# vpc-ccg/freddie

Hardware: AMD Instinct MI355X
Metric: reads segmented/sec (whole node) (higher is better)
Workload: dtype u32

## Files before the change

freddie_amd/_lib.py:

```python
import ctypes
import os

import numpy as np

from . import build as _build

_lib = None


class SegError(RuntimeError):

    def __init__(self, msg, code=None):
        super().__init__(msg)
        self.code = code


ERR_ARG, ERR_HIP, ERR_INPUT, ERR_UNSUPPORTED = 1, 2, 3, 4


class _Params(ctypes.Structure):
    _fields_ = [
        ("sigma", ctypes.c_double), ("threshold_rate", ctypes.c_double), ("variance_factor", ctypes.c_double),
        ("max_problem_size", ctypes.c_int32), ("min_read_support_outside", ctypes.c_int32),
        ("ignore_ends", ctypes.c_int32),
# ... 9 lines not shown
        ("part_iv_off", ctypes.c_void_p), ("iv_start", ctypes.c_void_p), ("iv_end", ctypes.c_void_p),
        ("part_rep_off", ctypes.c_void_p), ("rep_weight", ctypes.c_void_p), ("rep_exon_off", ctypes.c_void_p),
        ("ex_ts", ctypes.c_void_p), ("ex_te", ctypes.c_void_p),
    ]


class _Sizes(ctypes.Structure):
    _fields_ = [("n_final", ctypes.c_int64), ("label_bytes", ctypes.c_int64), ("n_cand", ctypes.c_int64),
                ("n_problems", ctypes.c_int64), ("n_positions", ctypes.c_int64), ("max_problem_size", ctypes.c_int64),
                ("max_problem_reads", ctypes.c_int64)]


class _Reads(ctypes.Structure):
    _fields_ = [("n_read", ctypes.c_int64)] + [(k, ctypes.c_void_p) for k in (
        "read_part", "read_rep", "strand", "seq_len", "seq_off", "read_q_off", "qs", "qe", "cig_off", "cig_op", "cig_len", "seq_classes")]


READS_DTYPES = dict(read_part=np.int32, read_rep=np.int32, strand=np.uint8, seq_len=np.int32, seq_off=np.int64, read_q_off=np.int64,
                    qs=np.int32, qe=np.int32, cig_off=np.int64, cig_op=np.uint8, cig_len=np.int32, seq_classes=np.uint32)


class _Annot(ctypes.Structure):
    _fields_ = [("n_read", ctypes.c_int64)] + [(k, ctypes.c_void_p) for k in (
        "gap_off", "gaps", "clip_off", "clips", "poly_off", "polys", "tail", "tok_off", "tok")]


EXPORTS = ["fseg_annotate", "fseg_annotation", "fseg_abi_version", "fseg_source_hash", "fseg_results", "fseg_results_packed", "fseg_create", "fseg_destroy", "fseg_last_error", "fseg_set_params", "fseg_upload",
           "fseg_run", "fseg_sync", "fseg_get_sizes", "fseg_download", "fseg_tap", "fseg_set_profiling",
           "fseg_n_stages", "fseg_stage_name", "fseg_stage_ms", "fseg_scoring_algorithmic_bytes"]

PATHS = ("small_batch", "tiny_on", "wave_on", "fuse_on", "key32", "thr_part", "label_packed", "n_solve0", "n_solve1", "n_solve2",
         "n_wide0", "n_wide1", "n_wide2", "n_tiny", "n_work", "dpw", "wide16", "known", "solve8", "tiny_kernel", "score", "arena_dp",
         "plan", "n_arena_prob", "n_score0", "n_score1", "n_score2", "hist16", "iv_threads", "smooth_r", "yraw16", "thr_chain",
         "lane_sort")

TAPS = dict(pos_off=(1, np.int64), y_raw=(2, np.int32), y=(3, np.float64), threshold=(4, np.float64),
            cand_off=(5, np.int64), cand_y=(6, np.int32), fixed=(7, np.uint8), chosen=(8, np.uint8),
            final_off=(9, np.int64), final_y=(10, np.int32), problems=(11, np.int32),
            lane_start=(12, np.int32), lane_pmax=(13, np.int32), lane_exons=(14, np.int64),
            lane_stream=(15, np.int32), exon_stream=(16, np.int32), sync=(17, np.int32), paths=(18, np.int32),
            hist_ranges=(19, np.int64))


def lib_path():
    return os.environ.get("FSEG_LIB") or _build.SEG_SO


def load():
    global _lib
    if _lib is not None:
        return _lib
    path = lib_path()
    if not os.path.exists(path):
        raise SegError("%s not found: build it first (freddie_amd.build.build_seg()); there is no CPU fallback" % path)
    L = ctypes.CDLL(path)
    vp = ctypes.c_void_p
    L.fseg_abi_version.restype = ctypes.c_int
    L.fseg_create.restype = ctypes.c_int
    L.fseg_create.argtypes = [ctypes.c_int, ctypes.POINTER(vp)]
    L.fseg_destroy.restype = None
    L.fseg_destroy.argtypes = [vp]
    L.fseg_last_error.restype = ctypes.c_char_p
    L.fseg_last_error.argtypes = [vp]
    L.fseg_set_params.restype = ctypes.c_int
    L.fseg_set_params.argtypes = [vp, ctypes.POINTER(_Params)]
    L.fseg_upload.restype = ctypes.c_int
    L.fseg_upload.argtypes = [vp, ctypes.POINTER(_Batch)]
# ... 184 lines not shown
```

freddie_amd/csrc/freddie_seg.hip:

```cpp
#include "seg_kernels.h"

using namespace fseg;

namespace {

template <typename T> struct DevBuf {
    T *p = nullptr;
    size_t cap = 0;
    static size_t bytes(size_t n) { return n * sizeof(T); }
};
template <> struct DevBuf<void> {
    void *p = nullptr;
    size_t cap = 0;
    static size_t bytes(size_t n) { return n; }
    template <typename U> U *as() const { return static_cast<U *>(p); }
};
template <typename T> size_t bytes_of(const DevBuf<T> &, size_t n) { return DevBuf<T>::bytes(n); }
struct NoCopy { NoCopy() = default; NoCopy(const NoCopy &) = delete; NoCopy &operator=(const NoCopy &) = delete; };
template <typename T> struct OwnDev : DevBuf<T>, NoCopy {
    ~OwnDev() { if (this->p) (void)hipFree(this->p); }
    hipError_t alloc(size_t bytes) { this->cap = bytes; return hipMalloc(&this->p, bytes); }
};
struct Slab : OwnDev<void> {};
template <typename T> struct Pinned : NoCopy {
// ... 25 lines not shown
                                        "interval_scoring", "dp", "refine", "final_positions", "labels", "graph_pre",
                                        "graph_post"};

enum : unsigned {
    SEG_PRE1 = 1u,
    SEG_PRE2 = 2u,
    SEG_SCORE = 4u,
    SEG_POST1 = 8u,
    SEG_POST2 = 16u,
    SEG_STATUS = 32u,
    SEG_ALL = 63u,
};

}

hipError_t fseg_sort_pairs(void *tmp, size_t *tmp_bytes, const unsigned long long *keys_in, unsigned long long *keys_out,
                           const int *vals_in, int *vals_out, size_t n, unsigned end_bit, hipStream_t stream);

struct fseg_ctx {
    int device = 0;
    hipStream_t stream = nullptr;
    std::string err;
    bool have_params = false, have_batch = false, ran = false, pending = false;
    bool fetched = false;
    fseg_params P{};
    std::vector<double> w_main, w_refine, h_table;
    int n_part = 0;
    i64 K = 0, R = 0, I = 0, NPOS = 0, LANES = 0;
    i64 max_part_pos = 0;
    int thr_part = -1;
    int hist16 = -1;
    bool hist_packed = false;
    int thr_chain = -1;
    int yraw16 = -1;
    bool yraw_narrow = false;
    i64 max_part_lanes = 0;
    int n_tiles = 0;
    bool expanded = false;
    std::vector<i64> part_iv_off, part_rep_off;
    Slab slab_in, slab_pos, slab_arena;
    Pinned<char> h_stage;
    Pinned<char> h_res;
    size_t res_off[4] = {0, 0, 0, 0};
    std::vector<i64> res_pfo;
    OwnDev<void> d_labels;
    OwnDev<unsigned> d_packed;
    int fetched_packed = -1;
    bool label_packed_ok = true;
    bool label_has2 = false;
    bool run_label_packed = false;
    bool labels_unpacked = false;
    OwnDev<void> d_sort_tmp;
    DevBuf<i64> d_part_iv_off, d_part_rep_off, d_part_lane_off, d_pos_off, d_rep_exon_off, d_hc_p0, d_rb_sum, d_rb_base;
    DevBuf<int> d_iv_start, d_iv_end, d_iv_part, d_rep_weight, d_ex_ts, d_ex_te, d_iv_tile0, d_blk_iv0, d_rb_part, d_rb_r0, d_rb_max, d_rb_cmax,
        d_hc_part, d_hc_n, d_hc_glo, d_hc_ghi;
    DevBuf<TileDesc> d_tile_desc;
    DevBuf<longlong2> d_lane_ex;
    DevBuf<int> d_lane_start, d_lane_pmax, d_val_a, d_val_b, d_rep_last;
    DevBuf<i64> d_hc_llo, d_hc_lhi, d_rb_esum, d_rb_ebase;
    DevBuf<u64> d_key_a, d_key_b;
    DevBuf<int2> d_lane_lx, d_lex;
    i64 max_rep_exons = 0;
    OwnDev<double> d_w_main, d_w_refine, d_h_table;
    OwnDev<int2> d_thr_tab;
    DevBuf<unsigned> d_bits;
    DevBuf<void> d_y_raw;
// ... 59 lines not shown
    bool prob_self_scan = false;
    i64 scan_single_max = 512;
    bool force_scan_stall = false;
    hipGraph_t graph[2] = {nullptr, nullptr};
    hipGraphExec_t graph_exec[2] = {nullptr, nullptr};
    bool profile_plain = false;
    int n_graphs = 0;
    bool last_sized = false;
    hipEvent_t ev_b[ST_COUNT] = {}, ev_e[ST_COUNT] = {};
    hipEvent_t ev_g[4] = {};
    float stage_ms[ST_REPORTED] = {};
    static constexpr int kSide = 3, kForkEvents = 32;
    hipStream_t side[kSide] = {};
    hipEvent_t fj[kForkEvents] = {};
    bool use_fork = true;
    bool force_key64 = false;
    bool wide_by_seen = false;
    char score_plan[32] = "gM|W|hB|gST";
    bool use_wave = true;
    bool use_fuse = true;
    int fuse_lanes = kFuseLanesDefault;
    bool wide_solve = true;
    bool fuse_on = true;
    bool counts_known = false;
    i64 n_solve[3] = {0, 0, 0}, n_cls_work[4] = {0, 0, 0, 0}, n_dp_cls[3] = {0, 0, 0}, n_arena_prob = 0, n_tiny = 0;
    i64 n_wide[3] = {0, 0, 0};
    i64 max_ln = 0;
    i64 tiny_from = 256;
    bool trace = false;
    bool force_global_sort = false;
    enum { PATH_SMALL_BATCH, PATH_TINY_ON, PATH_WAVE_ON, PATH_FUSE_ON, PATH_KEY32, PATH_THR_PART, PATH_LABEL_PACKED, PATH_N_SOLVE,
           PATH_N_WIDE = PATH_N_SOLVE + 3, PATH_N_TINY = PATH_N_WIDE + 3, PATH_N_WORK, PATH_DPW, PATH_WIDE16, PATH_KNOWN, PATH_SOLVE8,
           PATH_TINY_KERNEL, PATH_SCORE, PATH_ARENA_DP, PATH_PLAN, PATH_N_ARENA_PROB, PATH_N_SCORE, PATH_HIST16 = PATH_N_SCORE + 3, PATH_IV_THREADS,
           PATH_SMOOTH_R, PATH_YRAW16, PATH_THR_CHAIN, PATH_LANE_SORT, PATH_WORDS };
    int paths[PATH_WORDS] = {};
    OwnDev<void> d_an_in, d_an_work, d_an_out;
    Pinned<char> h_an_in, h_an;
    bool have_annot = false;
    fseg_annot annot{};
    ~fseg_ctx();
};

namespace {

int fail(fseg_ctx *c, int code, const char *fmt, ...) {
    char buf[512];
    va_list ap;
    va_start(ap, fmt);
    vsnprintf(buf, sizeof buf, fmt, ap);
    va_end(ap);
    if (c) c->err = buf;
    if (code == FSEG_ERR_HIP) (void)hipGetLastError();
    return code;
}
thread_local std::string g_create_error;

#define HIP_TRY(c, expr)                                                                         \
    do {                                                                                         \
        hipError_t e__ = (expr);                                                                 \
        if (e__ != hipSuccess) return fail((c), FSEG_ERR_HIP, "%s: %s", #expr, hipGetErrorString(e__)); \
    } while (0)
#define TRY(expr) do { int rc__ = (expr); if (rc__) return rc__; } while (0)

static bool g_ablate_dp = false;
static std::atomic<int> g_in_flight[64];
static std::atomic<int> g_live[64];
static std::atomic<const fseg_ctx *> g_owner[64];
// ... 326 lines not shown
    hipLaunchKernelGGL(k_prob_emit, dim3(pg), dim3(256), 0, s, st, c->d_cand_pn.p, c->d_cand_ll.p,
                       c->d_cand_ln.p, c->d_seg_iv.p, c->d_cand_off.p, prob_bs,
                       pr, c->prob_cap, c->d_work_pc.p, c->d_cls_items.p,
                       c->work_cap, c->d_dp_items.p, c->d_prob_desc.p, c->d_iv_start.p,
                       c->d_iv_part.p, c->d_part_lane_off.p, split, c->d_solve_items.p, c->d_solve_desc.p,
                       c->d_wide_items.p, c->d_wide_all.p, c->d_cand_wide.p,
                       dev_sync ? sw : (SyncWords *)nullptr, sync_gen);
    launch_fork_waiters();
    if (c->prob_cap > 0 && any_arena) {
        if (stage_events && do_score) { end(ST_SCORE_PREP); begin(ST_SCORE); score_begun = true; }
        const int cov_blocks = work_grid < 2048 ? work_grid : 2048;
        const int pt_blocks = c->small_batch ? grid_for(c->prob_cap, 1, 512) : 0;
        if (!pt_blocks)
            hipLaunchKernelGGL(k_pair_thresholds, dim3(grid_for(c->prob_cap, 1, 2048)), dim3(256), 0, s, st, pr,
                               c->d_prob_desc.p, c->prob_cap, c->d_cand_off.p, c->d_cand_y.p,
                               c->d_h_table.p, c->P.h_len,
                               c->P.threshold_rate, c->d_pair_thr.p, c->pair_cap, c->d_amb.p,
                               c->d_out.p, c->tri_cap);
        hipLaunchKernelGGL(k_cov, dim3(cov_blocks + pt_blocks), dim3(kLaneChunk), 0, s, st,
                           c->d_prob_desc.p, c->prob_cap, c->d_work_pc.p, c->work_cap, c->d_cand_off.p,
                           c->d_cand_y.p, c->d_iv_start.p, c->d_lane_lx.p,
                           c->d_lex.p,
                           c->d_cov.p, c->cov_cap, c->d_work_active.p,
                           cov_blocks, pr, c->d_h_table.p, c->P.h_len, c->P.threshold_rate, c->d_pair_thr.p,
                           c->pair_cap, c->d_amb.p, c->d_out.p, c->tri_cap);
    }
    if (!score_begun) end(ST_SCORE_PREP);
    }
    if (do_score && !score_begun) begin(ST_SCORE);
    int *const census = c->paths;
    if (do_score) {
        for (int w = 0; w < fseg_ctx::PATH_WORDS; ++w)
            if (w != fseg_ctx::PATH_THR_PART && w != fseg_ctx::PATH_LABEL_PACKED && w != fseg_ctx::PATH_ARENA_DP && w != fseg_ctx::PATH_HIST16 &&
                w != fseg_ctx::PATH_IV_THREADS && w != fseg_ctx::PATH_SMOOTH_R && w != fseg_ctx::PATH_YRAW16 && w != fseg_ctx::PATH_THR_CHAIN && w != fseg_ctx::PATH_LANE_SORT) census[w] = 0;
        census[fseg_ctx::PATH_SMALL_BATCH] = c->small_batch; census[fseg_ctx::PATH_TINY_ON] = c->tiny_on; census[fseg_ctx::PATH_WAVE_ON] = wave;
        census[fseg_ctx::PATH_FUSE_ON] = c->use_fuse && c->fuse_on; census[fseg_ctx::PATH_KNOWN] = known; census[fseg_ctx::PATH_PLAN] = plan != nullptr;
    }
    if (do_score && c->prob_cap > 0) {
        const bool sfork = any_arena;
        hipStream_t qt = (tiny_max > 0 && sfork) ? fork(2) : s;
#ifdef FSEG_SCORE_TIMING
#define FSEG_TARG , c->d_tacc.p
#else
#define FSEG_TARG
#endif
#ifndef FSEG_WG_SMALL
#define FSEG_WG_SMALL 4096
#endif
#ifndef FSEG_WG_MID
#define FSEG_WG_MID 2048
#endif
#ifndef FSEG_WG_TINY
#define FSEG_WG_TINY 4096
#endif
#define FSEG_LAUNCH_SCORE(Q, NMV, CLS, MAXWG)                                                                           \
        do { note_score(CLS);                                                                                                  \
        hipLaunchKernelGGL(k_score<NMV>, dim3(work_grid < (MAXWG) ? work_grid : (MAXWG)), dim3(ScoreCfg<NMV>::kThreads),  \
                           score_lds_for((NMV) == kNMax ? c->nm_big : (NMV), (NMV) + 1), Q, st, CLS,                                 \
                           ((NMV) == kNMax ? c->nm_big : (NMV)), pr, c->prob_cap, c->d_cls_items.p,              \
                           c->d_prob_desc.p, c->work_cap, c->d_cand_off.p,                         \
                           c->d_cand_y.p, c->d_work_active.p, c->d_cov.p,        \
                           c->cov_cap, c->d_pair_thr.p, c->pair_cap, c->d_out.p, c->tri_cap,      \
                           c->d_amb.p FSEG_TARG); } while (0)
        auto wide_n = [&](int cls, size_t cnt_bytes) -> i64 { return (known && cls >= 0 && cls < 3 && cnt_bytes == 2) ? c->n_wide[cls] : -1; };
#define FSEG_SOLVE_N(CNT, CLS, N_ITEMS) (wide_n(CLS, sizeof(CNT)) >= 0 ? wide_n(CLS, sizeof(CNT)) : (i64)(N_ITEMS))
#define FSEG_SOLVE_WIDE(CNT, CLS) (wide_n(CLS, sizeof(CNT)) >= 0 ? c->d_wide_items.p : (const int *)nullptr)
#define FSEG_SOLVE_ARGS(NMV, CNT, CLS)                                                                                      \
// ... 263 lines not shown
                       c->d_seg_prev.p, c->d_cand_y.p, c->d_pos_off.p, c->d_y_raw.as<COUNT>(), \
                       c->d_w_refine.p, c->P.radius_refine, c->P.sigma, c->d_g.p, c->d_pk.p, \
                       c->d_pf.p, c->d_kp.p, flag_final_bits)
    if (c->yraw_narrow) { FSEG_LAUNCH_REFINE(uint16_t); }
    else { FSEG_LAUNCH_REFINE(int); }
#undef FSEG_LAUNCH_REFINE
    end(ST_REFINE); begin(ST_FINAL);
    pos_counts(s, flag_final_bits);
    hipLaunchKernelGGL(k_scan_emit<kEmitPositions>, dim3(pos_grid), dim3(256), 0, s, flag_final_bits,
                       NPOS, bsum, gsum, scan_state + 2 * scan_nb, &st->n_final, c->d_final_off.p + K, &st->err, (const double *)nullptr, (double *)nullptr, K, c->d_pos_off.p,
                       c->d_iv_start.p, c->d_blk_iv0.p, c->d_final_y.p, c->d_final_pos.p,
                       c->d_final_off.p, 0, c->d_final_iv.p);
    hipLaunchKernelGGL(k_label_cols, dim3(grid_for(NPOS / 8 + 1, 256, 2048)), dim3(256), 0, s, K, c->d_final_off.p,
                       c->d_final_y.p, c->d_final_iv.p, c->d_iv_part.p, c->d_h_table.p, c->P.h_len,
                       c->P.threshold_rate, c->d_thr_tab.p, c->d_col_thr.p, c->d_col_zero.p,
                       c->d_part_has2.p, n_part, c->d_part_iv_off.p, c->d_part_rep_off.p,
                       c->d_label_off.p, st, c->label_cap);
    end(ST_FINAL);
    }
    if (do_post2) {
    begin(ST_LABEL);
    if (c->label_cap > 0) {
        c->run_label_packed = lab_packed; c->labels_unpacked = false;
        c->paths[fseg_ctx::PATH_LABEL_PACKED] = lab_packed;
        if (lab_packed) {
            const i64 n16 = sized ? (label_fill_bytes + 15) / 16 : labels_n16;
            if (n16 > 0)
                hipLaunchKernelGGL(k_clear, dim3(grid_for(n16 / 4 + 1, 256, 4096)), dim3(256), 0, s, (Status *)nullptr, c->d_packed.p, n16);
        } else if (!ride_fill) {
            const i64 n16 = sized ? (label_fill_bytes + 15) / 16 : labels_n16;
            if (n16 > 0)
                hipLaunchKernelGGL(k_label_zero, dim3(grid_for(n16 / 8 + 1, 256, 4096)), dim3(256), 0, s, c->d_labels.as<uint4>(), n16);
        }
        hipLaunchKernelGGL(k_label_reads, dim3(grid_for((i64)c->n_rep_blocks * kLabelSplit, 1, 65536)), dim3(256), 0, s, c->n_rep_blocks,
                           c->d_rb_part.p, c->d_rb_r0.p, c->d_label_off.p, c->label_cap, n_part,
                           c->d_part_iv_off.p, c->d_part_rep_off.p, c->d_final_off.p,
                           c->d_final_pos.p, c->d_col_thr.p, c->d_rep_exon_off.p,
                           c->d_ex_ts.p, c->d_ex_te.p, c->d_col_zero.p,
                           c->d_part_has2.p, c->d_labels.as<unsigned char>(), lab_packed ? c->d_packed.p : (unsigned *)nullptr);
    }
    end(ST_LABEL);
    }
    if (segs & SEG_STATUS) HIP_TRY(c, hipMemcpyAsync(c->h_status.p, st, sizeof(Status), hipMemcpyDeviceToHost, s));
    HIP_TRY(c, fj_err);
    HIP_TRY(c, hipGetLastError());
    return FSEG_OK;
}

hipError_t wait_stream(fseg_ctx *c) {
    const auto t0 = std::chrono::steady_clock::now();
    for (;;) {
        hipError_t e = hipStreamQuery(c->stream);
        if (e != hipErrorNotReady) { (void)hipGetLastError(); return e; }
        if (std::chrono::steady_clock::now() - t0 > std::chrono::milliseconds(2)) break;
    }
    (void)hipGetLastError();
    return hipStreamSynchronize(c->stream);
}

int check_prep(fseg_ctx *c) {
    if (c->prep_checked) return FSEG_OK;
    c->prep_checked = true;
    const PrepStatus &ps = *c->h_prep;
    if (!ps.err) return FSEG_OK;
    int q = 0;
    for (int i = 1; i < 4; ++i) if (((ps.err >> i) & 1u) && (!((ps.err >> q) & 1u) || ps.bad_rep[i] < ps.bad_rep[q])) q = i;
    if (!((ps.err >> q) & 1u)) for (q = 0; q < 4 && !((ps.err >> q) & 1u); ++q) {}
    const long long r = (long long)ps.bad_rep[q];
    c->have_batch = false;
    switch (1u << q) {
        case kPrepExonEnds: return fail(c, FSEG_ERR_INPUT, "rep %lld: exon with start >= end (py/freddie_segment.py:160)", r);
        case kPrepExonOrder: return fail(c, FSEG_ERR_INPUT, "rep %lld: exons out of order (py/freddie_segment.py:158)", r);
// ... 282 lines not shown
        {k_solve<kNMax, unsigned short, int, false>, solve_lds_for(kNMax, kNMax + 1, 2)},
        {k_solve<kNMax, unsigned short, i64, false>, solve_lds_for(kNMax, kNMax + 1, 2)},
        {k_solve<kNMax, unsigned char, int, true>, solve_lds_for(kNMax, kNMax + 1, 1)},
        {k_solve<kNMax, unsigned short, int, true>, solve_lds_for(kNMax, kNMax + 1, 2)},
        {k_dpw<kNMax, unsigned char, int, 64>, dpw_lds_for(kNMax, 4, 1)},
        {k_dpw<kNMax, unsigned short, int, 64>, dpw_lds_for(kNMax, 4, 2)},
        {k_dpw<kNMax, unsigned char, i64, 64>, dpw_lds_for(kNMax, 8, 1)},
        {k_dpw<kNMax, unsigned short, i64, 64>, dpw_lds_for(kNMax, 8, 2)},
        {k_dpw<kNMax, unsigned char, int, 512>, dpw_lds_for(kNMax, 4, 1)},
        {k_dpw<kNMax, unsigned short, int, 512>, dpw_lds_for(kNMax, 4, 2)},
        {k_dpw<kNMax, unsigned char, i64, 512>, dpw_lds_for(kNMax, 8, 1)},
        {k_dpw<kNMax, unsigned short, i64, 512>, dpw_lds_for(kNMax, 8, 2)},
        {k_dp_huge, kHugeDpLds},
    };
    for (const auto &a : lds_attrs) CREATE_TRY(hipFuncSetAttribute(a.fn, hipFuncAttributeMaxDynamicSharedMemorySize, (int)a.bytes));
#undef CREATE_TRY
    return hipSuccess;
}

bool env_flag(const char *name) { const char *v = getenv(name); return v && v[0] == '1'; }
bool env_off(const char *name) { const char *v = getenv(name); return v && v[0] == '0'; }
void env_tri(const char *name, int &out) { const char *v = getenv(name); if (v && (v[0] == '0' || v[0] == '1')) out = v[0] - '0'; }
bool env_int(const char *name, i64 &out) { const char *v = getenv(name); if (!v || !v[0]) return false; out = atoll(v); return true; }
const char *env_str(const char *name) { return getenv(name); }

void read_switches(fseg_ctx *c) {
    i64 v = 0;
    if (env_off("FSEG_DEV_SYNC")) c->dev_sync = false;
    if (env_flag("FSEG_LABEL_BYTES")) c->label_packed_ok = false;
    env_tri("FSEG_THR_PART", c->thr_part);
    env_tri("FSEG_THR_CHAIN", c->thr_chain);
    env_tri("FSEG_HIST16", c->hist16);
    env_tri("FSEG_YRAW16", c->yraw16);
    if (env_int("FSEG_SYNC_TICKS", v) && v > 0) c->sync_ticks = (unsigned)v;
    if (env_flag("FSEG_NO_GRAPH")) c->use_graph = false;
    if (env_flag("FSEG_NO_FORK")) c->use_fork = false;
    if (env_flag("FSEG_NO_FUSE")) c->use_fuse = false;
    if (env_flag("FSEG_NO_WAVE")) c->use_wave = false;
    if (env_flag("FSEG_FORCE_KEY64")) c->force_key64 = true;
    if (env_flag("FSEG_WIDE_BY_SEEN")) c->wide_by_seen = true;
    if (const char *s = env_str("FSEG_SPLIT_DP")) c->split_dp = atoi(s) & 15;
    if (const char *s = env_str("FSEG_SCORE_PLAN")) snprintf(c->score_plan, sizeof c->score_plan, "%s", s);
    {
        int seen[4] = {0, 0, 0, 0};
        static const char kinds[] = "BMST";
        for (const char *q = c->score_plan; *q; ++q) { const char *at = strchr(kinds, *q); if (at) ++seen[at - kinds]; }
        int bars = 0;
        for (const char *q = c->score_plan; *q; ++q) bars += *q == '|';
        if (seen[0] != 1 || seen[1] != 1 || seen[2] != 1 || seen[3] != 1 || bars > fseg_ctx::kSide) c->score_plan[0] = 0;
    }
    if (env_int("FSEG_FUSE_LANES", v) && v > 0 && v <= kFuseLanesWide) c->fuse_lanes = (int)v;
    if (env_flag("FSEG_NO_SIZED")) c->use_sized = false;
    if (env_flag("FSEG_TRACE")) c->trace = true;
    if (env_flag("FSEG_GLOBAL_SORT")) c->force_global_sort = true;
    if (env_flag("FSEG_FORCE_SCAN_STALL")) c->force_scan_stall = true;
    if (env_int("FSEG_TINY_FROM", v)) c->tiny_from = v;
    if (env_int("FSEG_SCAN_SINGLE_MAX", v)) c->scan_single_max = v;
}

}

fseg_ctx::~fseg_ctx() {
    (void)hipSetDevice(device);
    if (stream) (void)hipStreamSynchronize(stream);
    for (hipStream_t q : side) if (q) (void)hipStreamSynchronize(q);
    drop_graph(this);
// ... 934 lines not shown
```

freddie_amd/csrc/seg_common.h:

```cpp
#pragma once
#include <hip/hip_runtime.h>
#include <type_traits>
#include <hsa/hsa.h>
#include <hsa/hsa_ext_amd.h>
#include <chrono>
#include <algorithm>
#include <atomic>
#include <mutex>
#include <cmath>
#include <cstdarg>
#include <cstdio>
#include <cstdlib>
#include <cstring>
#include <string>
#include <vector>

#include "freddie_seg.h"

namespace fseg {


typedef long long i64;

typedef unsigned long long u64;
// ... 1320 lines not shown

constexpr size_t kHugeScoreLds = (size_t)(kNHuge * (kNHuge - 1) / 2) * 8 + (size_t)kHugeSub * (kNHuge + 1) * 4;


constexpr size_t kHugeDpLds = (size_t)(kNHuge * (kNHuge - 1) / 2) * (8 + 4 + 1) + 16;


constexpr int kGiantWgs = 64;

inline size_t giant_score_lds(int nm) { return (size_t)(2 * nm + kHugeSub * (nm + 1)) * 4; }

inline size_t giant_dp_lds(int nm) { return (size_t)nm * 4; }

inline size_t giant_scratch_bytes(int nm) {
    const size_t pairs = (size_t)nm * (nm - 1) / 2;
    return ((pairs * (8 + 4 + 2) + 255) & ~(size_t)255);
}


constexpr int kSegChunks = 4;


constexpr int kRefCap = 1024;

constexpr int kLabelCols = 1024;

#ifndef FSEG_LABEL_STAGE
#define FSEG_LABEL_STAGE 1024
#endif
constexpr int kLabelStage = FSEG_LABEL_STAGE;

constexpr int kLabelSplit = 4;


enum : unsigned { kPrepExonEnds = 1u, kPrepExonOrder = 2u, kPrepExonInterval = 4u, kPrepNoExons = 8u };

struct PrepStatus {
    unsigned err;
    unsigned pad;
    i64 bad_rep[4];
};


constexpr int kLaneSortMax = 2048;

constexpr int kLexChunk = 4096;

__device__ __forceinline__ void lex_copy_tile(int eb, int ne, i64 src0, int tot_e, i64 tile_e0, const int *__restrict__ ex_ts,
                                              const int *__restrict__ ex_te, int2 *__restrict__ lex, unsigned char *owner_s ,
                                              int *eb_s , i64 *src_s ) {
    eb_s[threadIdx.x] = eb; src_s[threadIdx.x] = src0;
    for (int c0 = 0; c0 < tot_e; c0 += kLexChunk) {
        __syncthreads();
        const int lo = max(eb, c0), hi = min(eb + ne, c0 + kLexChunk);
        for (int o = lo; o < hi; ++o) owner_s[o - c0] = (unsigned char)threadIdx.x;
        __syncthreads();
        const int end = min(tot_e, c0 + kLexChunk);
        for (int o = c0 + (int)threadIdx.x; o < end; o += 256) {
            const int u = owner_s[o - c0];
            const i64 src = src_s[u] + (o - eb_s[u]);
            lex[tile_e0 + o] = make_int2(ex_ts[src], ex_te[src]);
        }
    }
    __syncthreads();
}

// ... 12 lines not shown
```

freddie_amd/csrc/seg_kernels.h:

```cpp
#pragma once
#include "seg_common.h"

namespace fseg {

__global__ void __launch_bounds__(256) k_thr_table(const double *h_table, int h_len, double tau, int2 *tab);

template <int BITS, typename Out>
__global__ void __launch_bounds__(512) k_hist(int n_chunks, const int *chunk_part, const i64 *chunk_p0, const int *chunk_n,
                                              const int *chunk_glo, const int *chunk_ghi, const i64 *chunk_lane_lo,
                                              const i64 *chunk_lane_hi, const i64 *part_iv_off,
                                              const int *iv_start, const int *iv_end, const i64 *pos_off,
                                              const i64 *part_lane_off, const int2 *__restrict__ lane_lx, const int *lane_start,
                                              const int *lane_pmax, const int2 *__restrict__ lex,
                                              int ignore_ends, Out *y_raw, Status *st, u64 *zero_ptr, i64 zero_n);

template <int R, typename Count>
#ifndef FSEG_SMOOTH_OCC
#define FSEG_SMOOTH_OCC 6
#endif
__global__ void __launch_bounds__(kSmoothThreads, FSEG_SMOOTH_OCC) k_smooth(int n_tiles, const TileDesc *__restrict__ tiles,
                                                const Count *__restrict__ y_raw, const double *__restrict__ w_g, int radius_rt,
                                                double *y_out, unsigned *flag_pos, unsigned *flag_cand, int *blk_pre, int *tile_tot,
                                                int *tile_defer);

// ... 142 lines not shown

__global__ void __launch_bounds__(512) k_dp_giant(Status *st, const int *dp_items, ProblemArrays pr, const ProbDesc *desc,
                                                  i64 prob_cap, const int *cand_y, const unsigned *out_g, i64 tri_cap,
                                                  const unsigned *amb_g, const int2 *pair_thr, i64 pair_cap, int support,
                                                  unsigned char *chosen, int nm, unsigned char *scratch, i64 scratch_stride);

template <typename Count>
__global__ void k_segments(i64 K, const i64 *pos_off, const i64 *cand_off, const int *cand_y, const Count *__restrict__ y_raw,
                           const int *__restrict__ blk_pre, const int *tile_tot, const int *iv_tile0, const unsigned char *chosen, unsigned *final_flag, int *rseg_c, int *rseg_prev,
                           Status *st);

template <typename Count>
__global__ void __launch_bounds__(64) k_refine(const Status *st, const int *cand_iv, const int *rseg_c,
                                               const int *rseg_prev, const int *cand_y, const i64 *pos_off,
                                               const Count *y_raw, const double *w_g, int radius, double sigma,
                                               double *g_scr, int *pk_scr, unsigned char *flag_scr,
                                               unsigned char *keep_scr, unsigned *final_flag);

__global__ void __launch_bounds__(256) k_label_cols(i64 K, const i64 *final_off, const int *final_y, const int *final_iv, const int *iv_part,
                                                    const double *h_table, int h_len, double tau, const int2 *thr_tab, int2 *col_thr,
                                                    unsigned char *col_zero, int *part_has2, int n_part,
                                                    const i64 *part_iv_off, const i64 *part_rep_off, i64 *label_off,
                                                    Status *st, i64 label_cap);

__global__ void __launch_bounds__(256) k_label_zero(uint4 *labels16, i64 n16);

__global__ void __launch_bounds__(256) k_label_reads(int n_blocks, const int *rb_part, const int *rb_r0,
                                                     const i64 *label_off, i64 label_cap, int n_part,
                                                     const i64 *part_iv_off, const i64 *part_rep_off,
                                                     const i64 *final_off, const int *final_pos, const int2 *col_thr,
                                                     const i64 *rep_exon_off, const int *ex_ts, const int *ex_te,
                                                     const unsigned char *col_zero, const int *part_has2,
                                                     unsigned char *labels, unsigned *packed);
__global__ void __launch_bounds__(256) k_unpack_labels(const unsigned *__restrict__ packed, uint4 *__restrict__ labels16, i64 n16);

__global__ void __launch_bounds__(256) k_pack_labels(const uint4 *__restrict__ labels16, unsigned *__restrict__ packed, i64 n16);

__global__ void __launch_bounds__(256) k_prep_reps(int n_blocks, const int *rb_part, const int *rb_r0, const i64 *part_rep_off,
                                                   const i64 *part_iv_off, const int *iv_start, const int *iv_end,
                                                   const i64 *rep_exon_off, const int *ex_ts, const int *ex_te, u64 *key,
                                                   int *val, int *rep_last, PrepStatus *ps);

__global__ void __launch_bounds__(256) k_lanes(int n_part, const i64 *part_rep_off, const i64 *part_lane_off, const u64 *key_sorted,
                                               const int *val_sorted, const int *rep_weight, const int *rep_last,
                                               const i64 *rep_exon_off, longlong2 *lane_ex, int *lane_start, int *lane_pmax,
                                               int sort_here, const u64 *key_unsorted, const int *ex_ts, const int *ex_te,
                                               int2 *lane_lx, int2 *lex);

__global__ void __launch_bounds__(256) k_lane_blocks(int n_blocks, const int *rb_part, const int *rb_r0, const i64 *part_rep_off,
                                                     const int *val_sorted, const int *rep_weight, const int *rep_last,
                                                     i64 *rb_sum, int *rb_max, const i64 *rep_exon_off, i64 *rb_esum);

__global__ void __launch_bounds__(256) k_lane_block_scan(int n_part, int n_blocks, const int *rb_part, const i64 *part_lane_off,
                                                         const i64 *rb_sum, const int *rb_max, i64 *rb_base, int *rb_cmax,
                                                         const i64 *part_rep_off, const i64 *rep_exon_off, const i64 *rb_esum, i64 *rb_ebase);

__global__ void __launch_bounds__(256) k_lane_emit(int n_blocks, const int *rb_part, const int *rb_r0, const i64 *part_rep_off,
                                                   const u64 *key_sorted, const int *val_sorted, const int *rep_weight, const int *rep_last,
                                                   const i64 *rep_exon_off, const i64 *rb_base, const int *rb_cmax,
                                                   longlong2 *lane_ex, int *lane_start, int *lane_pmax, const i64 *rb_ebase,
                                                   const int *ex_ts, const int *ex_te, int2 *lane_lx, int2 *lex);

__global__ void __launch_bounds__(256) k_hist_ranges(int n_chunks, const int *hc_part, const int *hc_glo, const int *hc_ghi,
                                                     const i64 *part_lane_off, const int *lane_start, const int *lane_pmax,
                                                     i64 *hc_llo, i64 *hc_lhi);

// ... 44 lines not shown
```

freddie_amd/csrc/seg_tail.hip:

```cpp
#include "seg_kernels.h"

namespace fseg {

__device__ __forceinline__ int end_blocks(const int *yr, int a0, int a, int b0, int b) {
    int4u va[kSumBlock / 4], vb[kSumBlock / 4];
#pragma unroll
    for (int e = 0; e < kSumBlock / 4; ++e) { va[e] = *reinterpret_cast<const int4u *>(yr + a0 + 4 * e); vb[e] = *reinterpret_cast<const int4u *>(yr + b0 + 4 * e); }
    int tot = 0;
#pragma unroll
    for (int e = 0; e < kSumBlock / 4; ++e) {
        const int pa = a0 + 4 * e, pb = b0 + 4 * e;
        tot += (pb <= b ? vb[e].x : 0) + (pb + 1 <= b ? vb[e].y : 0) + (pb + 2 <= b ? vb[e].z : 0) + (pb + 3 <= b ? vb[e].w : 0);
        tot -= (pa < a ? va[e].x : 0) + (pa + 1 < a ? va[e].y : 0) + (pa + 2 < a ? va[e].z : 0) + (pa + 3 < a ? va[e].w : 0);
    }
    return tot;
}
__device__ __forceinline__ int end_blocks(const uint16_t *yr, int a0, int a, int b0, int b) {
    uint4u va[kSumBlock / 8], vb[kSumBlock / 8];
#pragma unroll
    for (int e = 0; e < kSumBlock / 8; ++e) { va[e] = *reinterpret_cast<const uint4u *>(yr + a0 + 8 * e); vb[e] = *reinterpret_cast<const uint4u *>(yr + b0 + 8 * e); }
    const int na = a - a0, nb = b - b0 + 1;
    auto first = [](unsigned w, int n) { return n >= 2 ? (w & 0xffffu) + (w >> 16) : (n == 1 ? w & 0xffffu : 0u); };
    unsigned tot_a = 0, tot_b = 0;
#pragma unroll
// ... 342 lines not shown
        i64 S = F - 1;
        if (S <= 0) continue;
        if ((i64)rb_r0[blk] + sub * (256 / kLabelSplit) >= part_rep_off[p + 1]) continue;
        const int *fp = final_pos + f0;
        const int2 *th = col_thr + f0;
        __syncthreads();
        if (S <= kLabelStage) {
            for (int x = threadIdx.x; x <= S; x += blockDim.x) fp_s[x] = fp[x];
            for (int x = threadIdx.x; x < S; x += blockDim.x) th_s[x] = th[x];
            fp = fp_s; th = th_s;
        }
        __syncthreads();
        i64 r = (i64)rb_r0[blk] + sub * (256 / kLabelSplit) + (threadIdx.x / kLabelSplit);
        const int q = threadIdx.x % kLabelSplit;
#ifdef FSEG_LAB_NOSEARCH
        if (fp[0] != -12345) continue;
#endif
        if (!packed && part_has2[p]) {
            if (r < part_rep_off[p + 1]) {
                unsigned char *row0 = labels + label_off[p] + (r - part_rep_off[p]) * S;
                const unsigned char *cz = col_zero + f0;
                for (i64 x = S * q / kLabelSplit; x < S * (q + 1) / kLabelSplit; ++x) row0[x] = cz[x];
            }
            __threadfence_block();
            __syncthreads();
        }
        if (r >= part_rep_off[p + 1]) continue;
        const i64 row_g0 = label_off[p] + (r - part_rep_off[p]) * S;
        unsigned char *row = labels + row_g0;
        unsigned acc = 0;
        i64 acc_w = -1;
        i64 e = rep_exon_off[r], e1 = rep_exon_off[r + 1];
        if (e >= e1) continue;
        int first_ts = ex_ts[e], last_te = ex_te[e1 - 1];
        int lo = 0, hi = (int)S;
        while (lo < hi) { int mid = (lo + hi) >> 1; if (fp[mid + 1] <= first_ts) lo = mid + 1; else hi = mid; }
        int c_hi = lo; hi = (int)S;
        while (c_hi < hi) { int mid = (c_hi + hi) >> 1; if (fp[mid] <= last_te) c_hi = mid + 1; else hi = mid; }
        const int span = c_hi - lo;
        const int c_a = lo + (int)((i64)span * q / kLabelSplit), c_b = lo + (int)((i64)span * (q + 1) / kLabelSplit);
        if (c_a >= c_b) continue;
#ifdef FSEG_LAB_NOLOOP
        if (c_a != -12345) { if (c_b == 0x7ffffff0) atomicOr(&packed[0], 1u); continue; }
#endif
        if (q) {
            const int g = fp[c_a];
            i64 a = e, b = e1;
            while (a < b) { i64 mid = (a + b) >> 1; if (ex_te[mid] < g) a = mid + 1; else b = mid; }
            e = a;
        }
        int ts = 0, te = 0;
        if (e < e1) { ts = ex_ts[e]; te = ex_te[e]; }
        for (int c = c_a; c < c_b; ++c) {
            int2 t2 = th[c];
            if (t2.x == 0x7fffffff) continue;
            int g0 = fp[c], g1 = fp[c + 1];
            while (e < e1 && te < g0) { ++e; if (e < e1) { ts = ex_ts[e]; te = ex_te[e]; } }
            int cov = 0;
            if (e < e1 && ts < g1) {
                int a = ts > g0 ? ts : g0, b2 = te + 1 < g1 ? te + 1 : g1;
                if (b2 > a) cov += b2 - a;
                for (i64 x = e + 1; x < e1 && ex_ts[x] < g1; ++x) {
                    int a3 = ex_ts[x] > g0 ? ex_ts[x] : g0;
                    int b3 = ex_te[x] + 1 < g1 ? ex_te[x] + 1 : g1;
                    if (b3 > a3) cov += b3 - a3;
                }
            }
            const unsigned char lab = cov >= t2.x ? '1' : (cov <= t2.y ? '0' : '2');
            if (lab != (t2.y < 0 ? '2' : '0')) {
                if (packed) {
                    const i64 g = row_g0 + c, w = g >> 4;
#ifdef FSEG_LAB_NOSTORE
                    if (w != acc_w) { acc_w = w; }
#else
                    if (w != acc_w) { if (acc) atomicOr(&packed[acc_w], acc); acc_w = w; acc = 0; }
#endif
                    acc |= (unsigned)(lab - '0') << (2 * (int)(g & 15));
                } else row[c] = lab;
            }
        }
        if (acc) atomicOr(&packed[acc_w], acc);
    }
}




__global__ void __launch_bounds__(256) k_unpack_labels(const unsigned *__restrict__ packed, uint4 *__restrict__ labels16, i64 n16) {
    for (i64 i = (i64)blockIdx.x * blockDim.x + threadIdx.x; i < n16; i += (i64)gridDim.x * blockDim.x) {
        const unsigned v = packed[i];
        unsigned w[4];
#pragma unroll
        for (int q = 0; q < 4; ++q) {
            const unsigned b = (v >> (8 * q)) & 0xffu;
            w[q] = 0x30303030u | (b & 3u) | ((b & 0xcu) << 6) | ((b & 0x30u) << 12) | ((b & 0xc0u) << 18);
        }
        labels16[i] = make_uint4(w[0], w[1], w[2], w[3]);
    }
}
__global__ void __launch_bounds__(256) k_pack_labels(const uint4 *__restrict__ labels16, unsigned *__restrict__ packed, i64 n16) {
    for (i64 i = (i64)blockIdx.x * blockDim.x + threadIdx.x; i < n16; i += (i64)gridDim.x * blockDim.x) {
        const uint4 v = labels16[i];
        const unsigned w[4] = {v.x, v.y, v.z, v.w};
        unsigned out = 0;
#pragma unroll
        for (int q = 0; q < 4; ++q) {
            const unsigned x = w[q] & 0x03030303u;
            out |= ((x & 3u) | ((x >> 6) & 0xcu) | ((x >> 12) & 0x30u) | ((x >> 18) & 0xc0u)) << (8 * q);
        }
        packed[i] = out;
    }
}

__attribute__((used)) static const void *const kInstances[] = {
    reinterpret_cast<const void *>(&k_segments<int>),
    reinterpret_cast<const void *>(&k_segments<uint16_t>),
    reinterpret_cast<const void *>(&k_refine<int>),
    reinterpret_cast<const void *>(&k_refine<uint16_t>),
// ... 4 lines not shown
```

Before: 626.8 million.

## Add LDS-staged label kernel caching exon intervals per read block

Adds k_label_reads_lds, which stages each unit's exon start/end pairs and per-read exon offsets in shared memory alongside the column positions and thresholds, then labels reads from LDS. It is selected by default via a tri-state env knob, with an optional grid-size cap. The aim is to replace repeated scattered global loads of exon arrays during the sweep and binary searches with shared-memory reads. This costs larger LDS use per block, which may lower occupancy, and adds an extra staging pass and barrier per unit.

```diff
diff --git a/freddie_amd/_lib.py b/freddie_amd/_lib.py
--- a/freddie_amd/_lib.py
+++ b/freddie_amd/_lib.py
@@ -65,7 +65,7 @@
 PATHS = ("small_batch", "tiny_on", "wave_on", "fuse_on", "key32", "thr_part", "label_packed", "n_solve0", "n_solve1", "n_solve2",
          "n_wide0", "n_wide1", "n_wide2", "n_tiny", "n_work", "dpw", "wide16", "known", "solve8", "tiny_kernel", "score", "arena_dp",
          "plan", "n_arena_prob", "n_score0", "n_score1", "n_score2", "hist16", "iv_threads", "smooth_r", "yraw16", "thr_chain",
-         "lane_sort")
+         "lane_sort", "label_lds")
 
 TAPS = dict(pos_off=(1, np.int64), y_raw=(2, np.int32), y=(3, np.float64), threshold=(4, np.float64),
             cand_off=(5, np.int64), cand_y=(6, np.int32), fixed=(7, np.uint8), chosen=(8, np.uint8),
diff --git a/freddie_amd/csrc/freddie_seg.hip b/freddie_amd/csrc/freddie_seg.hip
--- a/freddie_amd/csrc/freddie_seg.hip
+++ b/freddie_amd/csrc/freddie_seg.hip
@@ -81,6 +81,8 @@
     int hist16 = -1;
     bool hist_packed = false;
     int thr_chain = -1;
+    int label_lds = -1;
+    i64 label_grid = 0;
     int yraw16 = -1;
     bool yraw_narrow = false;
     i64 max_part_lanes = 0;
@@ -206,7 +208,7 @@
     enum { PATH_SMALL_BATCH, PATH_TINY_ON, PATH_WAVE_ON, PATH_FUSE_ON, PATH_KEY32, PATH_THR_PART, PATH_LABEL_PACKED, PATH_N_SOLVE,
            PATH_N_WIDE = PATH_N_SOLVE + 3, PATH_N_TINY = PATH_N_WIDE + 3, PATH_N_WORK, PATH_DPW, PATH_WIDE16, PATH_KNOWN, PATH_SOLVE8,
            PATH_TINY_KERNEL, PATH_SCORE, PATH_ARENA_DP, PATH_PLAN, PATH_N_ARENA_PROB, PATH_N_SCORE, PATH_HIST16 = PATH_N_SCORE + 3, PATH_IV_THREADS,
-           PATH_SMOOTH_R, PATH_YRAW16, PATH_THR_CHAIN, PATH_LANE_SORT, PATH_WORDS };
+           PATH_SMOOTH_R, PATH_YRAW16, PATH_THR_CHAIN, PATH_LANE_SORT, PATH_LABEL_LDS, PATH_WORDS };
     int paths[PATH_WORDS] = {};
     OwnDev<void> d_an_in, d_an_work, d_an_out;
     Pinned<char> h_an_in, h_an;
@@ -599,7 +601,7 @@
     if (do_score) {
         for (int w = 0; w < fseg_ctx::PATH_WORDS; ++w)
             if (w != fseg_ctx::PATH_THR_PART && w != fseg_ctx::PATH_LABEL_PACKED && w != fseg_ctx::PATH_ARENA_DP && w != fseg_ctx::PATH_HIST16 &&
-                w != fseg_ctx::PATH_IV_THREADS && w != fseg_ctx::PATH_SMOOTH_R && w != fseg_ctx::PATH_YRAW16 && w != fseg_ctx::PATH_THR_CHAIN && w != fseg_ctx::PATH_LANE_SORT) census[w] = 0;
+                w != fseg_ctx::PATH_IV_THREADS && w != fseg_ctx::PATH_SMOOTH_R && w != fseg_ctx::PATH_YRAW16 && w != fseg_ctx::PATH_THR_CHAIN && w != fseg_ctx::PATH_LANE_SORT && w != fseg_ctx::PATH_LABEL_LDS) census[w] = 0;
         census[fseg_ctx::PATH_SMALL_BATCH] = c->small_batch; census[fseg_ctx::PATH_TINY_ON] = c->tiny_on; census[fseg_ctx::PATH_WAVE_ON] = wave;
         census[fseg_ctx::PATH_FUSE_ON] = c->use_fuse && c->fuse_on; census[fseg_ctx::PATH_KNOWN] = known; census[fseg_ctx::PATH_PLAN] = plan != nullptr;
     }
@@ -929,12 +931,18 @@
             if (n16 > 0)
                 hipLaunchKernelGGL(k_label_zero, dim3(grid_for(n16 / 8 + 1, 256, 4096)), dim3(256), 0, s, c->d_labels.as<uint4>(), n16);
         }
-        hipLaunchKernelGGL(k_label_reads, dim3(grid_for((i64)c->n_rep_blocks * kLabelSplit, 1, 65536)), dim3(256), 0, s, c->n_rep_blocks,
-                           c->d_rb_part.p, c->d_rb_r0.p, c->d_label_off.p, c->label_cap, n_part,
-                           c->d_part_iv_off.p, c->d_part_rep_off.p, c->d_final_off.p,
-                           c->d_final_pos.p, c->d_col_thr.p, c->d_rep_exon_off.p,
-                           c->d_ex_ts.p, c->d_ex_te.p, c->d_col_zero.p,
-                           c->d_part_has2.p, c->d_labels.as<unsigned char>(), lab_packed ? c->d_packed.p : (unsigned *)nullptr);
+        const int lab_grid = grid_for((i64)c->n_rep_blocks * kLabelSplit, 1, c->label_grid > 0 && c->label_grid < 65536 ? c->label_grid : 65536);
+        c->paths[fseg_ctx::PATH_LABEL_LDS] = c->label_lds != 0;
+#define FSEG_LAUNCH_LABEL(KERNEL)                                                                                       \
+        hipLaunchKernelGGL(KERNEL, dim3(lab_grid), dim3(256), 0, s, c->n_rep_blocks,                                    \
+                           c->d_rb_part.p, c->d_rb_r0.p, c->d_label_off.p, c->label_cap, n_part,                        \
+                           c->d_part_iv_off.p, c->d_part_rep_off.p, c->d_final_off.p,                                   \
+                           c->d_final_pos.p, c->d_col_thr.p, c->d_rep_exon_off.p,                                       \
+                           c->d_ex_ts.p, c->d_ex_te.p, c->d_col_zero.p,                                                 \
+                           c->d_part_has2.p, c->d_labels.as<unsigned char>(), lab_packed ? c->d_packed.p : (unsigned *)nullptr)
+        if (c->label_lds != 0) { FSEG_LAUNCH_LABEL(k_label_reads_lds); }
+        else { FSEG_LAUNCH_LABEL(k_label_reads); }
+#undef FSEG_LAUNCH_LABEL
     }
     end(ST_LABEL);
     }
@@ -1283,6 +1291,8 @@
     env_tri("FSEG_THR_CHAIN", c->thr_chain);
     env_tri("FSEG_HIST16", c->hist16);
     env_tri("FSEG_YRAW16", c->yraw16);
+    env_tri("FSEG_LABEL_LDS", c->label_lds);
+    if (env_int("FSEG_LABEL_GRID", v) && v > 0) c->label_grid = v;
     if (env_int("FSEG_SYNC_TICKS", v) && v > 0) c->sync_ticks = (unsigned)v;
     if (env_flag("FSEG_NO_GRAPH")) c->use_graph = false;
     if (env_flag("FSEG_NO_FORK")) c->use_fork = false;
diff --git a/freddie_amd/csrc/seg_common.h b/freddie_amd/csrc/seg_common.h
--- a/freddie_amd/csrc/seg_common.h
+++ b/freddie_amd/csrc/seg_common.h
@@ -1376,6 +1376,12 @@
 
 constexpr int kLabelSplit = 4;
 
+constexpr int kLabelReps = 256 / kLabelSplit;
+#ifndef FSEG_LABEL_EXONS
+#define FSEG_LABEL_EXONS 960
+#endif
+constexpr int kLabelExons = FSEG_LABEL_EXONS;
+
 
 enum : unsigned { kPrepExonEnds = 1u, kPrepExonOrder = 2u, kPrepExonInterval = 4u, kPrepNoExons = 8u };
 
diff --git a/freddie_amd/csrc/seg_kernels.h b/freddie_amd/csrc/seg_kernels.h
--- a/freddie_amd/csrc/seg_kernels.h
+++ b/freddie_amd/csrc/seg_kernels.h
@@ -198,6 +198,13 @@
                                                      const i64 *rep_exon_off, const int *ex_ts, const int *ex_te,
                                                      const unsigned char *col_zero, const int *part_has2,
                                                      unsigned char *labels, unsigned *packed);
+__global__ void __launch_bounds__(256) k_label_reads_lds(int n_blocks, const int *rb_part, const int *rb_r0,
+                                                         const i64 *label_off, i64 label_cap, int n_part,
+                                                         const i64 *part_iv_off, const i64 *part_rep_off,
+                                                         const i64 *final_off, const int *final_pos, const int2 *col_thr,
+                                                         const i64 *rep_exon_off, const int *ex_ts, const int *ex_te,
+                                                         const unsigned char *col_zero, const int *part_has2,
+                                                         unsigned char *labels, unsigned *packed);
 __global__ void __launch_bounds__(256) k_unpack_labels(const unsigned *__restrict__ packed, uint4 *__restrict__ labels16, i64 n16);
 
 __global__ void __launch_bounds__(256) k_pack_labels(const uint4 *__restrict__ labels16, unsigned *__restrict__ packed, i64 n16);
diff --git a/freddie_amd/csrc/seg_tail.hip b/freddie_amd/csrc/seg_tail.hip
--- a/freddie_amd/csrc/seg_tail.hip
+++ b/freddie_amd/csrc/seg_tail.hip
@@ -398,7 +398,16 @@
         i64 acc_w = -1;
         i64 e = rep_exon_off[r], e1 = rep_exon_off[r + 1];
         if (e >= e1) continue;
-        int first_ts = ex_ts[e], last_te = ex_te[e1 - 1];
+#ifdef FSEG_LAB_NOEXON
+        const int fk_w = max(1, (fp[S] - fp[0]) / (int)S), fk_0 = fp[0] + 9 * fk_w * (int)(r & 63);
+        const i64 fk_e = e;
+#define LAB_TS(i) (fk_0 + 3 * fk_w * (int)((i) - fk_e))
+#define LAB_TE(i) (LAB_TS(i) + 2 * fk_w)
+#else
+#define LAB_TS(i) ex_ts[i]
+#define LAB_TE(i) ex_te[i]
+#endif
+        int first_ts = LAB_TS(e), last_te = LAB_TE(e1 - 1);
         int lo = 0, hi = (int)S;
         while (lo < hi) { int mid = (lo + hi) >> 1; if (fp[mid + 1] <= first_ts) lo = mid + 1; else hi = mid; }
         int c_hi = lo; hi = (int)S;
@@ -412,23 +421,23 @@
         if (q) {
             const int g = fp[c_a];
             i64 a = e, b = e1;
-            while (a < b) { i64 mid = (a + b) >> 1; if (ex_te[mid] < g) a = mid + 1; else b = mid; }
+            while (a < b) { i64 mid = (a + b) >> 1; if (LAB_TE(mid) < g) a = mid + 1; else b = mid; }
             e = a;
         }
         int ts = 0, te = 0;
-        if (e < e1) { ts = ex_ts[e]; te = ex_te[e]; }
+        if (e < e1) { ts = LAB_TS(e); te = LAB_TE(e); }
         for (int c = c_a; c < c_b; ++c) {
             int2 t2 = th[c];
             if (t2.x == 0x7fffffff) continue;
             int g0 = fp[c], g1 = fp[c + 1];
-            while (e < e1 && te < g0) { ++e; if (e < e1) { ts = ex_ts[e]; te = ex_te[e]; } }
+            while (e < e1 && te < g0) { ++e; if (e < e1) { ts = LAB_TS(e); te = LAB_TE(e); } }
             int cov = 0;
             if (e < e1 && ts < g1) {
                 int a = ts > g0 ? ts : g0, b2 = te + 1 < g1 ? te + 1 : g1;
                 if (b2 > a) cov += b2 - a;
-                for (i64 x = e + 1; x < e1 && ex_ts[x] < g1; ++x) {
-                    int a3 = ex_ts[x] > g0 ? ex_ts[x] : g0;
-                    int b3 = ex_te[x] + 1 < g1 ? ex_te[x] + 1 : g1;
+                for (i64 x = e + 1; x < e1 && LAB_TS(x) < g1; ++x) {
+                    int a3 = LAB_TS(x) > g0 ? LAB_TS(x) : g0;
+                    int b3 = LAB_TE(x) + 1 < g1 ? LAB_TE(x) + 1 : g1;
                     if (b3 > a3) cov += b3 - a3;
                 }
             }
@@ -447,9 +456,143 @@
         }
         if (acc) atomicOr(&packed[acc_w], acc);
     }
-}
-
-
+#undef LAB_TS
+#undef LAB_TE
+}
+
+
+
+
+
+struct LabelUnit { int n_rep; i64 e_base, n_ex; };
+__device__ __forceinline__ LabelUnit label_unit(i64 r0, i64 r_end, const i64 *rep_exon_off) {
+    LabelUnit u;
+    u.n_rep = (int)(r_end - r0 < kLabelReps ? r_end - r0 : kLabelReps);
+    u.e_base = rep_exon_off[r0];
+    u.n_ex = rep_exon_off[r0 + u.n_rep] - u.e_base;
+    return u;
+}
+__device__ __forceinline__ bool label_stage_exons(const LabelUnit &u, i64 r0, const i64 *rep_exon_off, const int *ex_ts, const int *ex_te,
+                                                  int *reo_s, int2 *ex_s) {
+    for (int x = threadIdx.x; x <= u.n_rep; x += blockDim.x) reo_s[x] = (int)(rep_exon_off[r0 + x] - u.e_base);
+    if (u.n_ex > kLabelExons) return false;
+    for (int x = threadIdx.x; x < (int)u.n_ex; x += blockDim.x) ex_s[x] = make_int2(ex_ts[u.e_base + x], ex_te[u.e_base + x]);
+    return true;
+}
+
+template <bool COLS_LDS, bool EXONS_LDS>
+__device__ __forceinline__ void label_rep(const int *fp_g, const int2 *th_g, const int *fp_s, const int2 *th_s, const int2 *ex_s,
+                                          const int *ts_g, const int *te_g, int e, const int e1, const int S, const int q,
+                                          const i64 row_g0, unsigned char *row, unsigned *packed) {
+    auto FP = [&](int i) -> int { if constexpr (COLS_LDS) return fp_s[i]; else return fp_g[i]; };
+    auto TH = [&](int i) -> int2 { if constexpr (COLS_LDS) return th_s[i]; else return th_g[i]; };
+    auto TS = [&](int i) -> int { if constexpr (EXONS_LDS) return ex_s[i].x; else return ts_g[i]; };
+    auto TE = [&](int i) -> int { if constexpr (EXONS_LDS) return ex_s[i].y; else return te_g[i]; };
+    unsigned acc = 0;
+    i64 acc_w = -1;
+    const int first_ts = TS(e), last_te = TE(e1 - 1);
+    int lo = 0, hi = S;
+    while (lo < hi) { int mid = (lo + hi) >> 1; if (FP(mid + 1) <= first_ts) lo = mid + 1; else hi = mid; }
+    int c_hi = lo; hi = S;
+    while (c_hi < hi) { int mid = (c_hi + hi) >> 1; if (FP(mid) <= last_te) c_hi = mid + 1; else hi = mid; }
+    const int span = c_hi - lo;
+    const int c_a = lo + (int)((i64)span * q / kLabelSplit), c_b = lo + (int)((i64)span * (q + 1) / kLabelSplit);
+    if (c_a >= c_b) return;
+    if (q) {
+        const int g = FP(c_a);
+        int a = e, b = e1;
+        while (a < b) { int mid = (a + b) >> 1; if (TE(mid) < g) a = mid + 1; else b = mid; }
+        e = a;
+    }
+    int ts = 0, te = 0;
+    if (e < e1) { ts = TS(e); te = TE(e); }
+    for (int c = c_a; c < c_b; ++c) {
+        const int2 t2 = TH(c);
+        if (t2.x == 0x7fffffff) continue;
+        const int g0 = FP(c), g1 = FP(c + 1);
+        while (e < e1 && te < g0) { ++e; if (e < e1) { ts = TS(e); te = TE(e); } }
+        int cov = 0;
+        if (e < e1 && ts < g1) {
+            int a = ts > g0 ? ts : g0, b2 = te + 1 < g1 ? te + 1 : g1;
+            if (b2 > a) cov += b2 - a;
+            for (int x = e + 1; x < e1; ++x) {
+                const int xs = TS(x);
+                if (!(xs < g1)) break;
+                const int xe = TE(x);
+                int a3 = xs > g0 ? xs : g0;
+                int b3 = xe + 1 < g1 ? xe + 1 : g1;
+                if (b3 > a3) cov += b3 - a3;
+            }
+        }
+        const unsigned char lab = cov >= t2.x ? '1' : (cov <= t2.y ? '0' : '2');
+        if (lab != (t2.y < 0 ? '2' : '0')) {
+            if (packed) {
+                const i64 g = row_g0 + c, w = g >> 4;
+                if (w != acc_w) { if (acc) atomicOr(&packed[acc_w], acc); acc_w = w; acc = 0; }
+                acc |= (unsigned)(lab - '0') << (2 * (int)(g & 15));
+            } else row[c] = lab;
+        }
+    }
+    if (acc) atomicOr(&packed[acc_w], acc);
+}
+
+__global__ void __launch_bounds__(256) k_label_reads_lds(int n_blocks, const int *rb_part, const int *rb_r0,
+                                                         const i64 *label_off, i64 label_cap, int n_part,
+                                                         const i64 *part_iv_off, const i64 *part_rep_off,
+                                                         const i64 *final_off, const int *final_pos, const int2 *col_thr,
+                                                         const i64 *rep_exon_off, const int *ex_ts, const int *ex_te,
+                                                         const unsigned char *col_zero, const int *part_has2,
+                                                         unsigned char *labels, unsigned *packed) {
+    __shared__ int fp_s[kLabelCols + 1];
+    __shared__ int2 th_s[kLabelCols];
+    __shared__ int2 ex_s[kLabelExons];
+    __shared__ int reo_s[kLabelReps + 1];
+    if (label_off[n_part] > label_cap) return;
+    for (i64 unit = blockIdx.x; unit < (i64)n_blocks * kLabelSplit; unit += gridDim.x) {
+        const int blk = (int)(unit / kLabelSplit), sub = (int)(unit % kLabelSplit);
+        const int p = rb_part[blk];
+        const i64 f0 = final_off[part_iv_off[p]];
+        const i64 S = final_off[part_iv_off[p + 1]] - f0 - 1;
+        if (S <= 0) continue;
+        const i64 r0 = (i64)rb_r0[blk] + sub * kLabelReps, r_end = part_rep_off[p + 1];
+        if (r0 >= r_end) continue;
+        const int *fp = final_pos + f0;
+        const int2 *th = col_thr + f0;
+        const LabelUnit u = label_unit(r0, r_end, rep_exon_off);
+        const bool cols_lds = S <= kLabelStage;
+        __syncthreads();
+        if (cols_lds) {
+            for (int x = threadIdx.x; x <= S; x += blockDim.x) fp_s[x] = fp[x];
+            for (int x = threadIdx.x; x < S; x += blockDim.x) th_s[x] = th[x];
+        }
+        const bool exons_lds = label_stage_exons(u, r0, rep_exon_off, ex_ts, ex_te, reo_s, ex_s);
+        __syncthreads();
+        const i64 r = r0 + (threadIdx.x / kLabelSplit);
+        const int q = threadIdx.x % kLabelSplit;
+        if (!packed && part_has2[p]) {
+            if (r < r_end) {
+                unsigned char *row0 = labels + label_off[p] + (r - part_rep_off[p]) * S;
+                const unsigned char *cz = col_zero + f0;
+                for (i64 x = S * q / kLabelSplit; x < S * (q + 1) / kLabelSplit; ++x) row0[x] = cz[x];
+            }
+            __threadfence_block();
+            __syncthreads();
+        }
+        if (r >= r_end) continue;
+        const int e = reo_s[threadIdx.x / kLabelSplit], e1 = reo_s[threadIdx.x / kLabelSplit + 1];
+        if (e >= e1) continue;
+        const i64 row_g0 = label_off[p] + (r - part_rep_off[p]) * S;
+        unsigned char *row = labels + row_g0;
+        const int *ts_g = ex_ts + u.e_base, *te_g = ex_te + u.e_base;
+        if (cols_lds) {
+            if (exons_lds) label_rep<true, true>(fp, th, fp_s, th_s, ex_s, ts_g, te_g, e, e1, (int)S, q, row_g0, row, packed);
+            else label_rep<true, false>(fp, th, fp_s, th_s, ex_s, ts_g, te_g, e, e1, (int)S, q, row_g0, row, packed);
+        } else {
+            if (exons_lds) label_rep<false, true>(fp, th, fp_s, th_s, ex_s, ts_g, te_g, e, e1, (int)S, q, row_g0, row, packed);
+            else label_rep<false, false>(fp, th, fp_s, th_s, ex_s, ts_g, te_g, e, e1, (int)S, q, row_g0, row, packed);
+        }
+    }
+}
 
 
 __global__ void __launch_bounds__(256) k_unpack_labels(const unsigned *__restrict__ packed, uint4 *__restrict__ labels16, i64 n16) {
```

Measured after the change: 655.1 million (median of 6 runs). +4.5%, better.
